# Starfish-develop/Starfish

Hardware: AMD Instinct MI355X
Metric: log-likelihood evals/sec, 4096-pixel order, batch=128 walkers (higher is better)
Workload: dtype f64; 1 GPU; cfg2: synthetic single order N_pix=4096, 8 eigenspectra, M=27, N_f=8192, 1 global + 1 local kernel, all 13 parameters thawed, batch=128 walkers per GPU; global_batch=128, units_per_gpu=128, parallelism=(order x walker) units sharded x1, one process per GPU, no data-path collective

## Files before the change

### starfish_amd/csrc/sf_chol_wide.h

```cpp
#pragma once
#include "sf_device.h"
#include "sf_chol_tile.h"
#include "sf_chol_panel.h"

#define WST (3 * GT * GK)
static constexpr size_t SF_PANELW_LDS = (3 * WST + 4 * GT) * sizeof(double);
struct sf_panelw_args {
    double* C;
    int64_t sC;
    int lda, n;
    int k0;
    int row0, nslab;
    int slab_step;
    const double* Wt0;
    const double* Wt1;
    int64_t sW;
    double* rhs;
    int ldr;
    double* Sout;
    int64_t sS;
    int ldS;
    const double* genY;
    const unsigned char* tilemap;
    int64_t sY;
    int ldy, mpad, nt128;
    int fp;
#ifdef SF_TUNING
    long long* stamps;
#endif
};
#ifdef SF_TUNING
#define SF_W_STAMP(i) do { if (g.stamps && blockIdx.x == gridDim.x / 2 && threadIdx.x == 0) g.stamps[i] = wall_clock64(); } while (0)
#else
#define SF_W_STAMP(i)
#endif

template <bool RHS>
__device__ __forceinline__ void sf_panelw_body(const sf_panelw_args& g, const int id, double* __restrict__ smw, const int tid) {
    constexpr int TM = 2, TN = 4;
    double* red = smw + 3 * WST;

    const int b = id / g.nslab;
    const int sl = id - b * g.nslab;
    const int row0 = g.row0 + sl * g.slab_step * GT;
    const int rows_here = min(GT, g.n - row0);
    const int k0 = g.k0;
    const int cfp = k0 == 0 ? g.fp : 0;

    const int lane = tid & 63;
    const int w = __builtin_amdgcn_readfirstlane(tid >> 6);
    const int wm = w & 3, wn = w >> 2;
    const int l15 = lane & 15, lq = lane >> 4;
    double* Cb = g.C + (int64_t)b * g.sC;
#define WBC(ni) ((((ni) >> 1) * GT) + wn * 32 + (((ni)&1) * 16))
    const bool wave_live = wm * 32 < rows_here;

    sf_d4 acc[TM][TN];
    SF_W_STAMP(0);
    {
        typedef __attribute__((address_space(3))) void* lds_ptr;
        const unsigned lds0 = (unsigned)(size_t)(lds_ptr)smw;
        const int grow = lane >> 3, gpos = lane & 7;
        unsigned soff[3];
        const double* sbase = sf_uniform_ptr(Cb + g.fp);
#pragma unroll
        for (int j = 0; j < 3; ++j) {
            const int G = 3 * w + j;
            const bool isA = G < 16;
            const int r = (isA ? G : G - 16) * 8 + grow;
            const int c = gpos ^ sf_swz(r);
            soff[j] = (unsigned)(((int64_t)(isA ? row0 + min(r, rows_here - 1) : k0 + r) * g.lda + 2 * c) * 8);
        }
        auto glds16 = [&](const double* sb, unsigned voff, unsigned lds_dst) {
            unsigned keep;
            asm volatile("s_mov_b32 %0, m0\n\ts_mov_b32 m0, %3\n\ts_nop 0\n\tglobal_load_lds_dwordx4 %1, %2\n\ts_mov_b32 m0, %0"
                         : "=&s"(keep)
                         : "v"(voff), "s"(sb), "s"(lds_dst)
                         : "memory");
        };
        auto gload = [&](int kt, int stage) {
#pragma unroll
            for (int j = 0; j < 3; ++j) glds16(sf_uniform_ptr(sbase + kt * GK), soff[j], lds0 + (unsigned)(stage * WST * 8 + (3 * w + j) * 1024));
        };
        auto gwait = [&]() { asm volatile("s_waitcnt vmcnt(0)" ::: "memory"); };
        const int nk = max(k0 - g.fp, 0) / GK;
        if (nk > 0) gload(0, 0);
        if (nk > 1) gload(1, 1);

        bool gen_half[2] = {false, false};
        if (g.tilemap) {
            const unsigned char* tm = g.tilemap + (int64_t)b * g.nt128 * g.nt128 + (row0 / GT) * g.nt128 + k0 / GT;
            gen_half[0] = !tm[0];
            gen_half[1] = !tm[1];
        }
#pragma unroll
        for (int hf = 0; hf < 2; ++hf) {
            if (gen_half[hf]) {
                const double* Yb = g.genY + (int64_t)b * g.sY;
                const int gr = row0 + wm * 32 + l15;
                const int gc = k0 + hf * GT + wn * 32 + l15;
#pragma unroll
                for (int mi = 0; mi < TM; ++mi)
#pragma unroll
                    for (int nn = 0; nn < 2; ++nn) acc[mi][2 * hf + nn] = (sf_d4){0.0, 0.0, 0.0, 0.0};
                for (int kk = 0; kk < g.mpad; kk += 8) {
                    double ya[2][TM], yb[2][2];
#pragma unroll
                    for (int u = 0; u < 2; ++u) {
                        const double* yk = Yb + (int64_t)(min(kk + 4 * u, g.mpad - 4) + lq) * g.ldy;
#pragma unroll
                        for (int i = 0; i < TM; ++i) ya[u][i] = yk[min(gr + i * 16, g.ldy + g.fp - 1)];
#pragma unroll
                        for (int i = 0; i < 2; ++i) yb[u][i] = gc + i * 16 >= cfp ? yk[min(gc + i * 16, g.ldy + g.fp - 1)] : 0.0;
                    }
#pragma unroll
                    for (int u = 0; u < 2; ++u) {
                        if (kk + 4 * u >= g.mpad) break;
#pragma unroll
                        for (int mi = 0; mi < TM; ++mi)
#pragma unroll
                            for (int nn = 0; nn < 2; ++nn)
                                acc[mi][2 * hf + nn] = __builtin_amdgcn_mfma_f64_16x16x4f64(ya[u][mi], yb[u][nn], acc[mi][2 * hf + nn], 0, 0, 0);
                    }
                }
            } else {
                const double* Cin = Cb + (int64_t)row0 * g.lda + k0;
#pragma unroll
                for (int mi = 0; mi < TM; ++mi)
#pragma unroll
                    for (int nn = 0; nn < 2; ++nn) {
                        const int col = WBC(2 * hf + nn) + l15;
#pragma unroll
                        for (int r = 0; r < 4; ++r) {
                            const int row = wm * 32 + mi * 16 + lq + 4 * r;
                            acc[mi][2 * hf + nn][r] = (row < rows_here && col >= cfp) ? Cin[(int64_t)row * g.lda + col] : 0.0;
                        }
                    }
            }
        }
        gwait();
        __syncthreads();
#pragma unroll
        for (int mi = 0; mi < TM; ++mi)
#pragma unroll
            for (int ni = 0; ni < TN; ++ni)
#pragma unroll
                for (int r = 0; r < 4; ++r) asm volatile("" : "+v"(acc[mi][ni][r]));
        SF_W_STAMP(1);

        const int sw = sf_swz(l15);
        const int e0 = 2 * ((2 * lq) ^ sw), e1 = 2 * ((2 * lq + 1) ^ sw);
        const int arow = (wm * 32 + l15) * GK, brow = (GT + wn * 32 + l15) * GK;
        auto frag = [&](int stage, int h, double2(&a)[TM], double2(&bb)[TN]) {
            const double* S = smw + stage * WST + (h ? e1 : e0);
#pragma unroll
            for (int i = 0; i < TM; ++i) a[i] = *(const double2*)(S + arow + i * 16 * GK);
#pragma unroll
            for (int i = 0; i < TN; ++i) bb[i] = *(const double2*)(S + brow + ((i >> 1) * GT + (i & 1) * 16) * GK);
        };
        auto mfma_part = [&](const double2(&a)[TM], const double2(&bb)[TN], auto lo_t, auto hi_t) {
            constexpr int lo = decltype(lo_t)::value, hi = decltype(hi_t)::value;
#pragma unroll
            for (int i = lo; i < hi; ++i) {
                const int y = i >> 3, mi = (i >> 2) & 1, ni = i & 3;
                acc[mi][ni] = __builtin_amdgcn_mfma_f64_16x16x4f64(y ? a[mi].y : a[mi].x, y ? bb[ni].y : bb[ni].x, acc[mi][ni], 0, 0, 1);
            }
        };
        typedef std::integral_constant<int, 0> I0;
        typedef std::integral_constant<int, 8> I8;
        typedef std::integral_constant<int, 16> I16;
        double2 a0[TM], b0[TN], a1[TM], b1[TN];
        int s0 = 0, s1 = 1, s2 = 2;
        if (nk > 0 && wave_live) frag(0, 0, a0, b0);
        for (int kt = 0; kt < nk; ++kt) {
            if (wave_live) {
                __builtin_amdgcn_s_setprio(1);
                mfma_part(a0, b0, I0(), I8());
                __builtin_amdgcn_s_setprio(0);
            }
            if (kt + 2 < nk) gload(kt + 2, s2);
            if (wave_live) {
                frag(s0, 1, a1, b1);
                __builtin_amdgcn_s_setprio(1);
                mfma_part(a0, b0, I8(), I16());
                __builtin_amdgcn_s_setprio(0);
                if (kt + 1 < nk) frag(s1, 0, a0, b0);
                __builtin_amdgcn_s_setprio(1);
                mfma_part(a1, b1, I0(), I16());
                __builtin_amdgcn_s_setprio(0);
            }
            gwait();
            __syncthreads();
            const int t = s0;
            s0 = s1;
            s1 = s2;
            s2 = t;
        }
    }

    double* Ach0 = smw;
    double* Bs = smw + 2 * GT * CLD;
    const int lr = tid >> 3, lc = (tid & 7) * 2;
    auto w_rows = [&](const double* Wt) { return Wt + (int64_t)b * g.sW + (int64_t)lr * SF_LDT + lc; };
    auto solve = [&](const double* Wt, double2 rw, auto nbtag) {
        constexpr int NB = decltype(nbtag)::value;
        const double* Wp = w_rows(Wt);
        int buf = 0;
#pragma unroll
        for (int sbi = 0; sbi < 8; ++sbi) {
            const int sb = 7 - sbi;
            double* Ach = Ach0 + ((sb >> 1) & 1) * (GT * CLD);
            if (sb == 7 && NB != 0) __syncthreads();
            if (sb & 1) {
                if (wn == (sb >> 1)) {
#pragma unroll
                    for (int nn = 0; nn < 2; ++nn)
#pragma unroll
                        for (int mi = 0; mi < TM; ++mi) {
#pragma unroll
                            for (int r = 0; r < 4; ++r)
                                Ach[(wm * 32 + mi * 16 + lq + 4 * r) * CLD + nn * 16 + l15] = acc[mi][NB + nn][r];
                            acc[mi][NB + nn] = (sf_d4){0.0, 0.0, 0.0, 0.0};
                        }
                }
            }
            {
                double* pb = Bs + buf * (GT * GLD) + lr * GLD + lc;
                pb[0] = rw.x;
                pb[1] = rw.y;
            }
            __syncthreads();
            if (sb > 0) rw = *(const double2*)(Wp + (sb - 1) * 16);
            if (sb <= 2 * wn + 1 && wave_live) {
                const double* Ab = Ach + (wm * 32 + l15) * CLD + (sb & 1) * 16 + lq;
                const double* Bb = Bs + buf * (GT * GLD) + (wn * 32 + l15) * GLD + lq;
#pragma unroll
                for (int ks = 0; ks < 4; ++ks) {
                    double a[TM], bb[2];
#pragma unroll
                    for (int i = 0; i < TM; ++i) a[i] = Ab[i * 16 * CLD + ks * 4];
#pragma unroll
                    for (int i = 0; i < 2; ++i) bb[i] = Bb[i * 16 * GLD + ks * 4];
#pragma unroll
                    for (int mi = 0; mi < TM; ++mi)
#pragma unroll
                        for (int nn = 0; nn < 2; ++nn)
                            acc[mi][NB + nn] = __builtin_amdgcn_mfma_f64_16x16x4f64(a[mi], bb[nn], acc[mi][NB + nn], 0, 0, 0);
                }
            }
            buf ^= 1;
        }
    };
    double2 rw0 = *(const double2*)(w_rows(g.Wt0) + 7 * 16);
    __syncthreads();
    SF_W_STAMP(2);
    solve(g.Wt0, rw0, std::integral_constant<int, 0>());
    SF_W_STAMP(3);
    double2 rw1 = *(const double2*)(w_rows(g.Wt1) + 7 * 16);

    {
        const double* L21 = Cb + (int64_t)(k0 + GT + lr) * g.lda + k0 + (tid & 7) * 4;
        auto l21 = [&](int q, double2& l0, double2& l1) {
            const bool real = (tid & 7) * 4 + q * 32 >= cfp;
            l0 = real ? *(const double2*)(L21 + q * 32) : make_double2(0.0, 0.0);
            l1 = real ? *(const double2*)(L21 + q * 32 + 2) : make_double2(0.0, 0.0);
        };
        double2 l0, l1, n0 = make_double2(0.0, 0.0), n1 = n0;
        l21(0, l0, l1);
#pragma unroll
        for (int q = 0; q < 4; ++q) {
            if (q + 1 < 4) l21(q + 1, n0, n1);
            double* Ach = Ach0 + (q & 1) * (GT * CLD);
            double* Bc = Bs + (q & 1) * (GT * CLD);
            if (q == 0) __syncthreads();
            if (wn == q) {
#pragma unroll
                for (int nn = 0; nn < 2; ++nn)
#pragma unroll
                    for (int mi = 0; mi < TM; ++mi)
#pragma unroll
                        for (int r = 0; r < 4; ++r)
                            Ach[(wm * 32 + mi * 16 + lq + 4 * r) * CLD + nn * 16 + l15] = acc[mi][nn][r];
            }
            {
                double* pb = Bc + lr * CLD + (tid & 7) * 4;
                pb[0] = l0.x;
                pb[1] = l0.y;
                pb[2] = l1.x;
                pb[3] = l1.y;
            }
            __syncthreads();
            if (wave_live) {
                const double* Ab = Ach + (wm * 32 + l15) * CLD + lq;
                const double* Bb = Bc + (wn * 32 + l15) * CLD + lq;
#pragma unroll
                for (int ks = 0; ks < 8; ++ks) {
                    double a[TM], bb[2];
#pragma unroll
                    for (int i = 0; i < TM; ++i) a[i] = Ab[i * 16 * CLD + ks * 4];
#pragma unroll
                    for (int i = 0; i < 2; ++i) bb[i] = Bb[i * 16 * CLD + ks * 4];
#pragma unroll
                    for (int mi = 0; mi < TM; ++mi)
#pragma unroll
                        for (int nn = 0; nn < 2; ++nn)
                            acc[mi][2 + nn] = __builtin_amdgcn_mfma_f64_16x16x4f64(a[mi], bb[nn], acc[mi][2 + nn], 0, 0, 1);
                }
            }
            l0 = n0;
            l1 = n1;
        }
    }
    SF_W_STAMP(4);
    solve(g.Wt1, rw1, std::integral_constant<int, 2>());
    SF_W_STAMP(5);
    constexpr int TLD = 130;
    const int nsb = wn == 0 ? 3 : 2;
    int sbi[3], sbj[3];
#pragma unroll
    for (int j = 0; j < 3; ++j) {
        const int t = min(wm + 4 * (wn + 4 * j), 35);
        int bi = 0;
        while ((bi + 1) * (bi + 2) / 2 <= t) ++bi;
        sbi[j] = bi;
        sbj[j] = t - bi * (bi + 1) / 2;
    }
    sf_d4 acc2[3];
    {
        const double* Sin = Cb + (int64_t)row0 * g.lda + row0;
        if (rows_here == GT) {
#pragma unroll
            for (int j = 0; j < 3; ++j)
#pragma unroll
                for (int r = 0; r < 4; ++r) {
                    const int row = 16 * sbi[j] + lq + 4 * r, col = 16 * sbj[j] + l15;
                    acc2[j][r] = Sin[(int64_t)row * g.lda + col];
                }
        } else {
#pragma unroll
            for (int j = 0; j < 3; ++j)
#pragma unroll
                for (int r = 0; r < 4; ++r) {
                    const int row = 16 * sbi[j] + lq + 4 * r, col = 16 * sbj[j] + l15;
                    acc2[j][r] = (j < nsb && row < rows_here && col < rows_here) ? Sin[(int64_t)row * g.lda + col] : 0.0;
                }
        }
    }
    double zc[TN] = {0.0, 0.0, 0.0, 0.0};
    if (RHS && g.rhs) {
        const double* z = g.rhs + (int64_t)b * g.ldr + k0;
#pragma unroll
        for (int ni = 0; ni < TN; ++ni) zc[ni] = WBC(ni) + l15 >= cfp ? z[WBC(ni) + l15] : 0.0;
    }

    {
        double* Lout = Cb + (int64_t)row0 * g.lda + k0;
#pragma unroll
        for (int mi = 0; mi < TM; ++mi)
#pragma unroll
            for (int ni = 0; ni < TN; ++ni) {
                const int col = WBC(ni) + l15;
#pragma unroll
                for (int r = 0; r < 4; ++r) {
                    const int row = wm * 32 + mi * 16 + lq + 4 * r;
                    if (row < rows_here && col >= cfp) Lout[(int64_t)row * g.lda + col] = acc[mi][ni][r];
                }
            }
        if (RHS && g.rhs) {
#pragma unroll
            for (int mi = 0; mi < TM; ++mi)
#pragma unroll
                for (int r = 0; r < 4; ++r) {
                    double v = 0.0;
#pragma unroll
                    for (int ni = 0; ni < TN; ++ni) v = __builtin_fma(acc[mi][ni][r], zc[ni], v);
                    v += __shfl_xor(v, 1);
                    v += __shfl_xor(v, 2);
                    v += __shfl_xor(v, 4);
                    v += __shfl_xor(v, 8);
                    if (l15 == 0) red[wn * GT + wm * 32 + mi * 16 + lq + 4 * r] = v;
                }
        }
    }

    SF_W_STAMP(6);
    {
        double* Ts = smw;
#pragma unroll
        for (int half = 0; half < 2; ++half) {
            __syncthreads();
#pragma unroll
            for (int nn = 0; nn < 2; ++nn)
#pragma unroll
                for (int mi = 0; mi < TM; ++mi)
#pragma unroll
                    for (int r = 0; r < 4; ++r)
                        Ts[(wm * 32 + mi * 16 + lq + 4 * r) * TLD + wn * 32 + nn * 16 + l15] = acc[mi][2 * half + nn][r];
            __syncthreads();
#pragma unroll
            for (int j = 0; j < 3; ++j) {
                if (j >= nsb) continue;
                const double* Pa = Ts + (sbi[j] * 16 + l15) * TLD + lq;
                const double* Pb = Ts + (sbj[j] * 16 + l15) * TLD + lq;
#pragma unroll 8
                for (int ks = 0; ks < GT / 4; ++ks)
                    acc2[j] = __builtin_amdgcn_mfma_f64_16x16x4f64(Pa[ks * 4], Pb[ks * 4], acc2[j], 0, 0, 1);
            }
        }
        SF_W_STAMP(7);
        const bool parked = g.Sout && sl == 0;
        double* So = parked ? g.Sout + (int64_t)b * g.sS : Cb + (int64_t)row0 * g.lda + row0;
        const int ldo = parked ? g.ldS : g.lda;
        if (rows_here == GT) {
#pragma unroll
            for (int j = 0; j < 2; ++j)
#pragma unroll
                for (int r = 0; r < 4; ++r) {
                    const int row = 16 * sbi[j] + lq + 4 * r, col = 16 * sbj[j] + l15;
                    So[(int64_t)row * ldo + col] = acc2[j][r];
                }
            if (nsb == 3) {
#pragma unroll
                for (int r = 0; r < 4; ++r) {
                    const int row = 16 * sbi[2] + lq + 4 * r, col = 16 * sbj[2] + l15;
                    So[(int64_t)row * ldo + col] = acc2[2][r];
                }
            }
        } else {
#pragma unroll
            for (int j = 0; j < 3; ++j) {
                if (j >= nsb) continue;
#pragma unroll
                for (int r = 0; r < 4; ++r) {
                    const int row = 16 * sbi[j] + lq + 4 * r, col = 16 * sbj[j] + l15;
                    if (row < rows_here && col < rows_here) So[(int64_t)row * ldo + col] = acc2[j][r];
                }
            }
        }
    }
    if (RHS && g.rhs) {
        if (tid < rows_here)
            g.rhs[(int64_t)b * g.ldr + row0 + tid] -= (red[tid] + red[GT + tid]) + (red[2 * GT + tid] + red[3 * GT + tid]);
    }
#ifdef SF_TUNING
    if (g.stamps) {
        __syncthreads();
        asm volatile("s_waitcnt vmcnt(0)" ::: "memory");
        SF_W_STAMP(8);
    }
#endif
#undef WBC
}
template <bool RHS>
__global__ __launch_bounds__(1024) void k_chol_panel_w(sf_panelw_args g) {
    extern __shared__ __attribute__((aligned(16))) double smw[];
    sf_panelw_body<RHS>(g, sf_xcd_remap(blockIdx.x, gridDim.x), smw, threadIdx.x);
}
#undef SF_W_STAMP
#undef WST
```

Before: 2758 evals/s.

## Double-buffer syrk transpose staging in quarters with vectorized LDS loads

```diff
diff --git a/starfish_amd/csrc/sf_chol_wide.h b/starfish_amd/csrc/sf_chol_wide.h
--- a/starfish_amd/csrc/sf_chol_wide.h
+++ b/starfish_amd/csrc/sf_chol_wide.h
@@ -314,7 +314,6 @@
     SF_W_STAMP(4);
     solve(g.Wt1, rw1, std::integral_constant<int, 2>());
     SF_W_STAMP(5);
-    constexpr int TLD = 130;
     const int nsb = wn == 0 ? 3 : 2;
     int sbi[3], sbj[3];
 #pragma unroll
@@ -385,27 +384,59 @@
 
     SF_W_STAMP(6);
     {
-        double* Ts = smw;
-#pragma unroll
-        for (int half = 0; half < 2; ++half) {
-            __syncthreads();
+        constexpr int QLD = GT / 2 + 4, NG = GT / 2 / 16;
+        auto dump = [&](int q) {
+            if ((wn >> 1) != (q & 1)) return;
+            double* Tq = smw + (q & 1) * (GT * QLD);
 #pragma unroll
             for (int nn = 0; nn < 2; ++nn)
 #pragma unroll
                 for (int mi = 0; mi < TM; ++mi)
 #pragma unroll
                     for (int r = 0; r < 4; ++r)
-                        Ts[(wm * 32 + mi * 16 + lq + 4 * r) * TLD + wn * 32 + nn * 16 + l15] = acc[mi][2 * half + nn][r];
-            __syncthreads();
+                        Tq[(wm * 32 + mi * 16 + lq + 4 * r) * QLD + (wn & 1) * 32 + nn * 16 + l15] = acc[mi][2 * (q >> 1) + nn][r];
+        };
+        const int lo = l15 * QLD + 2 * lq;
+        auto ld = [&](const double* T, int j, int gi, double2(&a)[2], double2(&bb)[2]) {
+            const double* Pa = T + sbi[j] * (16 * QLD) + lo + gi * 16;
+            const double* Pb = T + sbj[j] * (16 * QLD) + lo + gi * 16;
+            a[0] = *(const double2*)Pa;
+            a[1] = *(const double2*)(Pa + 8);
+            bb[0] = *(const double2*)Pb;
+            bb[1] = *(const double2*)(Pb + 8);
+        };
+        auto mm = [&](int j, const double2(&a)[2], const double2(&bb)[2]) {
+            __builtin_amdgcn_s_setprio(1);
+            acc2[j] = __builtin_amdgcn_mfma_f64_16x16x4f64(a[0].x, bb[0].x, acc2[j], 0, 0, 1);
+            acc2[j] = __builtin_amdgcn_mfma_f64_16x16x4f64(a[0].y, bb[0].y, acc2[j], 0, 0, 1);
+            acc2[j] = __builtin_amdgcn_mfma_f64_16x16x4f64(a[1].x, bb[1].x, acc2[j], 0, 0, 1);
+            acc2[j] = __builtin_amdgcn_mfma_f64_16x16x4f64(a[1].y, bb[1].y, acc2[j], 0, 0, 1);
+            __builtin_amdgcn_s_setprio(0);
+        };
+        __syncthreads();
+        dump(0);
+        __syncthreads();
+#pragma unroll
+        for (int q = 0; q < 4; ++q) {
+            if (q + 1 < 4) dump(q + 1);
+            const double* T = smw + (q & 1) * (GT * QLD);
+            double2 a0[2], b0[2], a1[2], b1[2];
+            ld(T, 0, 0, a0, b0);
 #pragma unroll
             for (int j = 0; j < 3; ++j) {
-                if (j >= nsb) continue;
-                const double* Pa = Ts + (sbi[j] * 16 + l15) * TLD + lq;
-                const double* Pb = Ts + (sbj[j] * 16 + l15) * TLD + lq;
-#pragma unroll 8
-                for (int ks = 0; ks < GT / 4; ++ks)
-                    acc2[j] = __builtin_amdgcn_mfma_f64_16x16x4f64(Pa[ks * 4], Pb[ks * 4], acc2[j], 0, 0, 1);
-            }
+                if (j >= nsb) break;
+#pragma unroll
+                for (int gi = 0; gi < NG; gi += 2) {
+                    ld(T, j, gi + 1, a1, b1);
+                    mm(j, a0, b0);
+                    if (gi + 2 < NG)
+                        ld(T, j, gi + 2, a0, b0);
+                    else if (j + 1 < 3 && j + 1 < nsb)
+                        ld(T, j + 1 < 3 ? j + 1 : 2, 0, a0, b0);
+                    mm(j, a1, b1);
+                }
+            }
+            if (q + 1 < 4) __syncthreads();
         }
         SF_W_STAMP(7);
         const bool parked = g.Sout && sl == 0;
```

Measured after the change: 2776 evals/s, median of 6. Within noise of the previous version (+0.6%).
